# jiangzhengkai/mxdetection

Measured on AMD Instinct MI355X. Metric: images/sec (whole node) Faster R-CNN R50-FPN 3x800x1333, higher is better.
Workload: dtype bf16; 1 GPU; Faster R-CNN ResNet-50-FPN bf16 train step, batch 2/GPU, 3x800x1333 (padded 1344); global_batch=2, parallelism=dp1, frozen=stem+C2, frozen BN folded, optimizer=SGD momentum 0.9 wd 1e-4, launch=hipGraph replay, input=resident, wgrad_side_stream=True, rpn_branch_stream=True, grouped_wgrad=True, filter_prefetch_hints=True, params_trainable=41538304

## Files before the change

mxdetection_amd/csrc/boxes.hip:

```cpp
#include "common.h"

namespace mxdet {

__global__ void box_iou_kernel(const float4* __restrict__ a, int64_t na, const float4* __restrict__ b,
                               int64_t nb, float* __restrict__ out) {
  int64_t idx = (int64_t)blockIdx.x * blockDim.x + threadIdx.x;
  if (idx >= na * nb) return;
  int64_t i = idx / nb, j = idx - i * nb;
  float4 p = a[i], q = b[j];
  out[idx] = mxdet_iou(p.x, p.y, p.z, p.w, q.x, q.y, q.z, q.w);
}

__global__ void anchors_kernel(const float* __restrict__ base, int A, int H, int W, int stride,
                               float4* __restrict__ out) {
  int64_t idx = (int64_t)blockIdx.x * blockDim.x + threadIdx.x;
  int64_t total = (int64_t)H * W * A;
  if (idx >= total) return;
  int a = (int)(idx % A);
  int64_t cell = idx / A;
  int x = (int)(cell % W), y = (int)(cell / W);
  float sx = (float)(x * stride), sy = (float)(y * stride);
  float4 o;
  o.x = base[a * 4 + 0] + sx;
  o.y = base[a * 4 + 1] + sy;
  o.z = base[a * 4 + 2] + sx;
  o.w = base[a * 4 + 3] + sy;
  out[idx] = o;
}

__global__ void fpn_level_kernel(const float* __restrict__ rois, int64_t R, int lvl_min, int lvl_max,
                                 int32_t* __restrict__ levels) {
  int64_t i = (int64_t)blockIdx.x * blockDim.x + threadIdx.x;
  if (i >= R) return;
  const float* r = rois + i * 5;
  int k = mxdet_fpn_level(r[1], r[2], r[3], r[4]);
  k = k < lvl_min ? lvl_min : (k > lvl_max ? lvl_max : k);
  levels[i] = k;
}

__global__ void __launch_bounds__(64)
nms_mask_kernel(const float4* __restrict__ boxes, const int32_t* __restrict__ counts, int n_max,
                int nwords_max, float thresh, unsigned long long* __restrict__ mask) {
  const int col_blk = blockIdx.x, row_blk = blockIdx.y, b = blockIdx.z;
  if (col_blk < row_blk) return;
  int n = counts[b];
  n = n > n_max ? n_max : n;
  if (row_blk * 64 >= n || col_blk * 64 >= n) return;
  __shared__ float4 cb[64];
  const int t = threadIdx.x;
  const float4* bx = boxes + (int64_t)b * n_max;
  int cj = col_blk * 64 + t;
  if (cj < n) cb[t] = bx[cj];
  __syncthreads();
  int i = row_blk * 64 + t;
  if (i >= n) return;
  float4 r = bx[i];
  int ncol = n - col_blk * 64;
  ncol = ncol > 64 ? 64 : ncol;
  unsigned long long bits = 0;
  for (int j = 0; j < ncol; ++j) {
    int c = col_blk * 64 + j;
    float4 q = cb[j];
    float v = mxdet_iou(r.x, r.y, r.z, r.w, q.x, q.y, q.z, q.w);
    if (c > i && v > thresh) bits |= (1ull << j);
  }
  mask[((int64_t)b * n_max + i) * nwords_max + col_blk] = bits;
}

__device__ __forceinline__ unsigned long long readlane64(unsigned long long v, int lane) {
  unsigned lo = (unsigned)v, hi = (unsigned)(v >> 32);
  lo = (unsigned)__builtin_amdgcn_readlane((int)lo, lane);
  hi = (unsigned)__builtin_amdgcn_readlane((int)hi, lane);
  return ((unsigned long long)hi << 32) | lo;
}

__global__ void __launch_bounds__(64)
nms_scan_kernel(const unsigned long long* __restrict__ mask, const int32_t* __restrict__ counts,
                const uint8_t* __restrict__ invalid, int n_max, int nwords_max, int max_keep,
                int32_t* __restrict__ keep_idx, int32_t* __restrict__ num_keep) {
  __shared__ unsigned long long rem[64];
  const int b = blockIdx.x, lane = threadIdx.x;
  int n = counts[b];
  n = n > n_max ? n_max : n;
  n = __builtin_amdgcn_readfirstlane(n);
  const int nw = (n + 63) >> 6;
  const unsigned long long* m = mask + (int64_t)b * n_max * nwords_max;
  for (int w = 0; w < nw; ++w) {
    int idx = w * 64 + lane;
    bool bad = (idx >= n) || (invalid != nullptr && invalid[(int64_t)b * n_max + idx] != 0);
    unsigned long long bm = __ballot(bad);
    if (lane == 0) rem[w] = bm;
  }
  __syncthreads();
  unsigned long long mykeep = 0;
  unsigned long long diag_next = (nw > 0 && lane < n) ? m[(int64_t)lane * nwords_max] : 0ull;
  for (int w = 0; w < nw; ++w) {
    const unsigned long long diag = diag_next;
    if (w + 1 < nw) {
      int row = (w + 1) * 64 + lane;
      diag_next = (row < n) ? m[(int64_t)row * nwords_max + (w + 1)] : 0ull;
    }
    __syncthreads();
    unsigned long long cur = rem[w];
    cur = readlane64(cur, 0);
    unsigned long long keepbits = 0;
    for (int bb = 0; bb < 64; ++bb) {
      unsigned long long d = readlane64(diag, bb);
      if (!((cur >> bb) & 1ull)) {
        keepbits |= (1ull << bb);
        cur |= d;
      }
    }
    if (lane == w) mykeep = keepbits;
    if ((keepbits >> lane) & 1ull) {
      const unsigned long long* row = m + (int64_t)(w * 64 + lane) * nwords_max;
      for (int j = w + 1; j < nw; ++j) {
        unsigned long long v = row[j];
        if (v) atomicOr(&rem[j], v);
      }
    }
  }
  int cnt = __popcll(mykeep);
  int incl = cnt;
  for (int off = 1; off < 64; off <<= 1) {
    int v = __shfl_up(incl, off);
    if (lane >= off) incl += v;
  }
  int excl = incl - cnt;
  int total = __shfl(incl, 63);
  unsigned long long kb = mykeep;
  int pos = excl;
  while (kb) {
    int bb = __ffsll((long long)kb) - 1;
    kb &= kb - 1;
    if (pos < max_keep) keep_idx[(int64_t)b * n_max + pos] = lane * 64 + bb;
    ++pos;
  }
  if (lane == 0) num_keep[b] = total < max_keep ? total : max_keep;
}

template <int NW>
__global__ void __launch_bounds__(64)
nms_scan_rows_kernel(const unsigned long long* __restrict__ mask, const int32_t* __restrict__ counts,
                     const uint8_t* __restrict__ invalid, int n_max, int nwords_max, int max_keep,
                     int32_t* __restrict__ keep_idx, int32_t* __restrict__ num_keep) {
  __shared__ unsigned long long rows[2][64][NW + 1];
  const int b = blockIdx.x, lane = threadIdx.x;
  int n = counts[b];
  n = n > n_max ? n_max : n;
  n = __builtin_amdgcn_readfirstlane(n);
  const int nw = (n + 63) >> 6;
  const unsigned long long* m = mask + (int64_t)b * n_max * NW;
  unsigned long long myrem = 0ull;
  for (int w = 0; w < nw; ++w) {
    int idx = w * 64 + lane;
    bool bad = (idx >= n) || (invalid != nullptr && invalid[(int64_t)b * n_max + idx] != 0);
    unsigned long long bm = __ballot(bad);
    if (lane == w) myrem = bm;
  }
  unsigned long long nxt[NW];
  auto load_row = [&](unsigned long long (&r)[NW], int w) {
    const unsigned long long* bp = m + (int64_t)(w * 64) * NW + lane;
#pragma unroll
    for (int k = 0; k < NW; ++k) r[k] = bp[k * 64];
  };
  auto stage = [&](const unsigned long long (&r)[NW], int buf, int w) {
    unsigned long long* dst = &rows[buf][lane >> 5][lane & 31];
#pragma unroll
    for (int k = 0; k < NW; ++k) dst[k * 2 * (NW + 1)] = r[k];
  };
  load_row(nxt, 0);
  stage(nxt, 0, 0);
  __syncthreads();
  const int myword = lane < NW ? lane : 0;
  unsigned long long mykeep = 0;
  int buf = 0;
  for (int w = 0; w < nw; ++w) {
#ifndef NMS_ABL_NOLOAD
    if (w + 1 < nw) load_row(nxt, w + 1);
#endif
    const unsigned long long diag = rows[buf][lane][w];
    unsigned long long c = readlane64(myrem, w);
#ifndef NMS_ABL_NOCHAIN
#pragma unroll
    for (int bb = 0; bb < 64; ++bb) {
      unsigned long long d = readlane64(diag, bb);
      c |= ((c >> bb) & 1ull) ? 0ull : d;
    }
#else
    c |= readlane64(diag, 0);
#endif
    const unsigned long long keepbits = ~c;
    if (lane == w) mykeep = keepbits;
    const unsigned klo = __builtin_amdgcn_readfirstlane((unsigned)keepbits);
    const unsigned khi = __builtin_amdgcn_readfirstlane((unsigned)(keepbits >> 32));
    unsigned long long acc = 0ull;
#ifndef NMS_ABL_NOOR
#pragma unroll
#else
    if (klo == 0x12345u)
#endif
    for (int ch = 0; ch < 8; ++ch) {
      const unsigned bits = ((ch < 4 ? klo : khi) >> (8 * (ch & 3))) & 0xffu;
      if (bits == 0u) continue;
      unsigned long long v[8];
#pragma unroll
      for (int t = 0; t < 8; ++t) v[t] = rows[buf][8 * ch + t][myword];
#pragma unroll
      for (int t = 0; t < 8; ++t) acc |= ((bits >> t) & 1u) ? v[t] : 0ull;
    }
    if (lane > w && lane < nw) myrem |= acc;
    if (w + 1 < nw) stage(nxt, buf ^ 1, w + 1);
    __syncthreads();
    buf ^= 1;
  }
  int cnt = __popcll(mykeep);
  int incl = cnt;
  for (int off = 1; off < 64; off <<= 1) {
    int v = __shfl_up(incl, off);
    if (lane >= off) incl += v;
  }
  int excl = incl - cnt;
  int total = __shfl(incl, 63);
  unsigned long long kb = mykeep;
  int pos = excl;
  while (kb) {
    int bb = __ffsll((long long)kb) - 1;
    kb &= kb - 1;
    if (pos < max_keep) keep_idx[(int64_t)b * n_max + pos] = lane * 64 + bb;
    ++pos;
  }
  if (lane == 0) num_keep[b] = total < max_keep ? total : max_keep;
}

}

using namespace mxdet;

extern "C" int mxdet_box_iou(const float* boxes_a, int64_t na, const float* boxes_b, int64_t nb,
                             float* out, mxdet_stream_t stream) {
  clear_error();
  MXDET_REQUIRE(na >= 0 && nb >= 0, MXDET_ESHAPE, "box_iou: negative size");
  if (na == 0 || nb == 0) return MXDET_OK;
  MXDET_REQUIRE(boxes_a && boxes_b && out, MXDET_EINVAL, "box_iou: null pointer");
  int64_t total = na * nb;
  hipLaunchKernelGGL(box_iou_kernel, dim3((unsigned)ceil_div<int64_t>(total, 256)), dim3(256), 0,
                     as_stream(stream), (const float4*)boxes_a, na, (const float4*)boxes_b, nb, out);
  return check_launch("box_iou");
}

extern "C" int mxdet_generate_anchors(const float* base_anchors, int32_t A, int32_t H, int32_t W,
                                      int32_t stride, float* out, mxdet_stream_t stream) {
  clear_error();
  MXDET_REQUIRE(A > 0 && H >= 0 && W >= 0 && stride > 0, MXDET_ESHAPE, "generate_anchors: bad shape");
  int64_t total = (int64_t)H * W * A;
  if (total == 0) return MXDET_OK;
  MXDET_REQUIRE(base_anchors && out, MXDET_EINVAL, "generate_anchors: null pointer");
  hipLaunchKernelGGL(anchors_kernel, dim3((unsigned)ceil_div<int64_t>(total, 256)), dim3(256), 0,
                     as_stream(stream), base_anchors, A, H, W, stride, (float4*)out);
  return check_launch("generate_anchors");
}

extern "C" int mxdet_fpn_level_map(const float* rois, int64_t R, int32_t lvl_min, int32_t lvl_max,
                                   int32_t* levels, mxdet_stream_t stream) {
  clear_error();
  MXDET_REQUIRE(R >= 0 && lvl_min <= lvl_max, MXDET_ESHAPE, "fpn_level_map: bad arguments");
  if (R == 0) return MXDET_OK;
  MXDET_REQUIRE(rois && levels, MXDET_EINVAL, "fpn_level_map: null pointer");
  hipLaunchKernelGGL(fpn_level_kernel, dim3((unsigned)ceil_div<int64_t>(R, 256)), dim3(256), 0,
                     as_stream(stream), rois, R, lvl_min, lvl_max, levels);
  return check_launch("fpn_level_map");
}

extern "C" size_t mxdet_nms_batched_workspace_bytes(int32_t B, int32_t n_max) {
  if (B <= 0 || n_max <= 0) return 0;
  size_t nwords = (size_t)(n_max + 63) / 64;
  if (nwords <= 32) nwords = 32;
  return ((size_t)B * n_max + 64) * nwords * sizeof(unsigned long long);
}

extern "C" int mxdet_nms_batched(const float* boxes, const int32_t* counts, const uint8_t* invalid,
                                 int32_t B, int32_t n_max, float thresh, int32_t max_keep,
                                 int32_t* keep_idx, int32_t* num_keep, void* workspace,
                                 size_t workspace_bytes, mxdet_stream_t stream) {
  clear_error();
  MXDET_REQUIRE(B >= 0 && n_max >= 0, MXDET_ESHAPE, "nms_batched: negative size");
  if (B == 0) return MXDET_OK;
  MXDET_REQUIRE(n_max <= 4096, MXDET_ESHAPE, "nms_batched: n_max %d > 4096 unsupported", n_max);
  MXDET_REQUIRE(counts && num_keep, MXDET_EINVAL, "nms_batched: null pointer");
  if (n_max == 0) {
    hipError_t e = zero_async(num_keep, sizeof(int32_t) * B, as_stream(stream));
    MXDET_REQUIRE(e == hipSuccess, MXDET_EHIP, "nms_batched: memset failed");
    return MXDET_OK;
  }
  MXDET_REQUIRE(boxes && keep_idx, MXDET_EINVAL, "nms_batched: null pointer");
  size_t need = mxdet_nms_batched_workspace_bytes(B, n_max);
  MXDET_REQUIRE(workspace && workspace_bytes >= need, MXDET_EWORKSPACE,
                "nms_batched: workspace %zu < %zu", workspace_bytes, need);
  int nwords = (n_max + 63) / 64;
  const int pitch = nwords <= 32 ? 32 : nwords;
  hipLaunchKernelGGL(nms_mask_kernel, dim3(nwords, nwords, B), dim3(64), 0, as_stream(stream),
                     (const float4*)boxes, counts, n_max, pitch, thresh,
                     (unsigned long long*)workspace);
  if (nwords <= 32)
    hipLaunchKernelGGL(nms_scan_rows_kernel<32>, dim3(B), dim3(64), 0, as_stream(stream),
                       (const unsigned long long*)workspace, counts, invalid, n_max, nwords,
                       max_keep < 0 ? 0 : max_keep, keep_idx, num_keep);
  else
    hipLaunchKernelGGL(nms_scan_kernel, dim3(B), dim3(64), 0, as_stream(stream),
                       (const unsigned long long*)workspace, counts, invalid, n_max, nwords,
                       max_keep < 0 ? 0 : max_keep, keep_idx, num_keep);
  return check_launch("nms_batched");
}
```

Baseline: 471.8 images/sec.

## Speed up batched NMS with division-free IoU filter and four-wave scan

The NMS mask kernel now precomputes box areas and classifies most pairs with a division-free comparison of intersection against threshold-scaled union, using slightly widened bounds. Only pairs too close to the threshold fall back to the exact IoU. The scan kernel grows from one wave to four: wave 0 resolves the diagonal word with a split 32-bit chain plus DPP reduction, and all four waves share row loading and the OR-accumulation through shared memory. This adds block-wide barriers per word and extra shared memory, in exchange for less per-pair arithmetic and more parallel bandwidth in a step that is a small part of the training iteration.

```diff
diff --git a/mxdetection_amd/csrc/boxes.hip b/mxdetection_amd/csrc/boxes.hip
--- a/mxdetection_amd/csrc/boxes.hip
+++ b/mxdetection_amd/csrc/boxes.hip
@@ -38,32 +38,73 @@
   levels[i] = k;
 }
 
+__device__ __forceinline__ float vmax(float a, float b) {
+  float r;
+  asm("v_max_f32 %0, %1, %2" : "=v"(r) : "v"(a), "v"(b));
+  return r;
+}
+__device__ __forceinline__ float vmin(float a, float b) {
+  float r;
+  asm("v_min_f32 %0, %1, %2" : "=v"(r) : "v"(a), "v"(b));
+  return r;
+}
+
+__device__ __forceinline__ float nms_fast_area(float4 p) {
+  const float w = p.z - p.x + 1.0f, h = p.w - p.y + 1.0f;
+  const float lim = 1073741824.0f;
+  const bool ok = w > 0.0f && h > 0.0f && fabsf(p.x) <= lim && fabsf(p.y) <= lim && fabsf(p.z) <= lim && fabsf(p.w) <= lim;
+  return ok ? w * h : __builtin_nanf("");
+}
+
 __global__ void __launch_bounds__(64)
 nms_mask_kernel(const float4* __restrict__ boxes, const int32_t* __restrict__ counts, int n_max,
-                int nwords_max, float thresh, unsigned long long* __restrict__ mask) {
+                int nwords_max, float thresh, float t_hi, float t_lo, unsigned long long* __restrict__ mask) {
   const int col_blk = blockIdx.x, row_blk = blockIdx.y, b = blockIdx.z;
   if (col_blk < row_blk) return;
   int n = counts[b];
   n = n > n_max ? n_max : n;
   if (row_blk * 64 >= n || col_blk * 64 >= n) return;
   __shared__ float4 cb[64];
+  __shared__ float ca[64];
   const int t = threadIdx.x;
   const float4* bx = boxes + (int64_t)b * n_max;
   int cj = col_blk * 64 + t;
-  if (cj < n) cb[t] = bx[cj];
+  const float4 cq = cj < n ? bx[cj] : make_float4(0.0f, 0.0f, 0.0f, 0.0f);
+  cb[t] = cq;
+  ca[t] = nms_fast_area(cq);
   __syncthreads();
   int i = row_blk * 64 + t;
   if (i >= n) return;
-  float4 r = bx[i];
+  const float4 r = bx[i];
+  const float ar = nms_fast_area(r);
   int ncol = n - col_blk * 64;
   ncol = ncol > 64 ? 64 : ncol;
-  unsigned long long bits = 0;
-  for (int j = 0; j < ncol; ++j) {
-    int c = col_blk * 64 + j;
-    float4 q = cb[j];
-    float v = mxdet_iou(r.x, r.y, r.z, r.w, q.x, q.y, q.z, q.w);
-    if (c > i && v > thresh) bits |= (1ull << j);
-  }
+  auto half = [&](int j0) -> unsigned {
+    unsigned set = 0u, open = 0u;
+#pragma unroll 8
+    for (int j = 0; j < 32; ++j) {
+      const float4 q = cb[j0 + j];
+      const float iw = fmaxf(vmin(r.z, q.z) - vmax(r.x, q.x) + 1.0f, 0.0f);
+      const float ih = fmaxf(vmin(r.w, q.w) - vmax(r.y, q.y) + 1.0f, 0.0f);
+      const float inter = iw * ih;
+      float ua = ar + ca[j0 + j];
+      ua = ua - inter;
+      const bool above = inter > t_hi * ua, below = inter < t_lo * ua;
+      set |= above ? (1u << j) : 0u;
+      open |= (above || below) ? 0u : (1u << j);
+    }
+    while (open) {
+      const int j = __ffs((int)open) - 1;
+      open &= open - 1u;
+      const float4 q = cb[j0 + j];
+      if (mxdet_iou(r.x, r.y, r.z, r.w, q.x, q.y, q.z, q.w) > thresh) set |= 1u << j;
+    }
+    return set;
+  };
+  const unsigned lo = half(0), hi = half(32);
+  unsigned long long bits = ((unsigned long long)hi << 32) | lo;
+  if (col_blk == row_blk) bits &= ~((2ull << t) - 1ull);
+  if (ncol < 64) bits &= (1ull << ncol) - 1ull;
   mask[((int64_t)b * n_max + i) * nwords_max + col_blk] = bits;
 }
 
@@ -139,81 +180,125 @@
   if (lane == 0) num_keep[b] = total < max_keep ? total : max_keep;
 }
 
+__device__ __forceinline__ unsigned long long resolve_word(unsigned long long c, unsigned long long diag, int lane) {
+  const unsigned dlo = (unsigned)diag, dhi = (unsigned)(diag >> 32);
+  unsigned clo = (unsigned)c, chi = (unsigned)(c >> 32);
+#ifndef NMS_ABL_NOCHAIN
+#pragma unroll
+  for (int bb = 0; bb < 32; ++bb) {
+    const unsigned d = (unsigned)__builtin_amdgcn_readlane((int)dlo, bb);
+    clo |= ((clo >> bb) & 1u) ? 0u : d;
+  }
+  int v = (int)((lane < 32 && !((clo >> lane) & 1u)) ? dhi : 0u);
+  v |= __builtin_amdgcn_update_dpp(0, v, 0x128, 0xf, 0xf, false);
+  v |= __builtin_amdgcn_update_dpp(0, v, 0x124, 0xf, 0xf, false);
+  v |= __builtin_amdgcn_update_dpp(0, v, 0x122, 0xf, 0xf, false);
+  v |= __builtin_amdgcn_update_dpp(0, v, 0x121, 0xf, 0xf, false);
+  chi |= (unsigned)__builtin_amdgcn_readlane(v, 0) | (unsigned)__builtin_amdgcn_readlane(v, 16);
+#pragma unroll
+  for (int bb = 0; bb < 32; ++bb) {
+    const unsigned d = (unsigned)__builtin_amdgcn_readlane((int)dhi, 32 + bb);
+    chi |= ((chi >> bb) & 1u) ? 0u : d;
+  }
+#else
+  clo |= (unsigned)__builtin_amdgcn_readlane((int)dlo, 0);
+  chi |= (unsigned)__builtin_amdgcn_readlane((int)dhi, 0);
+#endif
+  return ((unsigned long long)chi << 32) | clo;
+}
+
 template <int NW>
-__global__ void __launch_bounds__(64)
+__global__ void __launch_bounds__(256)
 nms_scan_rows_kernel(const unsigned long long* __restrict__ mask, const int32_t* __restrict__ counts,
                      const uint8_t* __restrict__ invalid, int n_max, int nwords_max, int max_keep,
                      int32_t* __restrict__ keep_idx, int32_t* __restrict__ num_keep) {
+  static_assert(NW % 4 == 0 && 256 % NW == 0 && NW <= 64, "four waves share the 64 x NW words of a run evenly");
   __shared__ unsigned long long rows[2][64][NW + 1];
-  const int b = blockIdx.x, lane = threadIdx.x;
+  __shared__ unsigned long long part[3][64];
+  __shared__ unsigned long long kept_word;
+  __shared__ unsigned long long removed0[NW];
+  const int b = blockIdx.x, tid = threadIdx.x, lane = tid & 63;
+  const int wave = __builtin_amdgcn_readfirstlane(tid >> 6);
   int n = counts[b];
   n = n > n_max ? n_max : n;
   n = __builtin_amdgcn_readfirstlane(n);
   const int nw = (n + 63) >> 6;
   const unsigned long long* m = mask + (int64_t)b * n_max * NW;
-  unsigned long long myrem = 0ull;
-  for (int w = 0; w < nw; ++w) {
-    int idx = w * 64 + lane;
-    bool bad = (idx >= n) || (invalid != nullptr && invalid[(int64_t)b * n_max + idx] != 0);
-    unsigned long long bm = __ballot(bad);
-    if (lane == w) myrem = bm;
-  }
-  unsigned long long nxt[NW];
-  auto load_row = [&](unsigned long long (&r)[NW], int w) {
-    const unsigned long long* bp = m + (int64_t)(w * 64) * NW + lane;
-#pragma unroll
-    for (int k = 0; k < NW; ++k) r[k] = bp[k * 64];
+  constexpr int NQ = NW / 4;
+  unsigned long long nxt[NQ];
+  auto load_row = [&](unsigned long long (&r)[NQ], int w) {
+    const unsigned long long* bp = m + (int64_t)(w * 64) * NW + tid;
+#pragma unroll
+    for (int k = 0; k < NQ; ++k) r[k] = bp[k * 256];
   };
-  auto stage = [&](const unsigned long long (&r)[NW], int buf, int w) {
-    unsigned long long* dst = &rows[buf][lane >> 5][lane & 31];
-#pragma unroll
-    for (int k = 0; k < NW; ++k) dst[k * 2 * (NW + 1)] = r[k];
+  auto stage = [&](const unsigned long long (&r)[NQ], int buf) {
+    unsigned long long* dst = &rows[buf][tid / NW][tid % NW];
+#pragma unroll
+    for (int k = 0; k < NQ; ++k) dst[k * (256 / NW) * (NW + 1)] = r[k];
   };
   load_row(nxt, 0);
-  stage(nxt, 0, 0);
+  uint8_t flag[NQ];
+#pragma unroll
+  for (int k = 0; k < NQ; ++k) flag[k] = 0;
+  if (invalid != nullptr) {
+    const uint8_t* inv = invalid + (int64_t)b * n_max;
+#pragma unroll
+    for (int k = 0; k < NQ; ++k) {
+      const int idx = (wave * NQ + k) * 64 + lane;
+      flag[k] = inv[idx < n ? idx : 0];
+    }
+  }
+#pragma unroll
+  for (int k = 0; k < NQ; ++k) {
+    const int idx = (wave * NQ + k) * 64 + lane;
+    const unsigned long long bm = __ballot(idx >= n || flag[k] != 0);
+    if (lane == 0) removed0[wave * NQ + k] = bm;
+  }
+  stage(nxt, 0);
   __syncthreads();
   const int myword = lane < NW ? lane : 0;
+  const unsigned long long myrem0 = removed0[myword];
+  unsigned long long myrem = lane < nw ? myrem0 : 0ull;
   unsigned long long mykeep = 0;
   int buf = 0;
   for (int w = 0; w < nw; ++w) {
 #ifndef NMS_ABL_NOLOAD
     if (w + 1 < nw) load_row(nxt, w + 1);
 #endif
-    const unsigned long long diag = rows[buf][lane][w];
-    unsigned long long c = readlane64(myrem, w);
-#ifndef NMS_ABL_NOCHAIN
-#pragma unroll
-    for (int bb = 0; bb < 64; ++bb) {
-      unsigned long long d = readlane64(diag, bb);
-      c |= ((c >> bb) & 1ull) ? 0ull : d;
-    }
-#else
-    c |= readlane64(diag, 0);
-#endif
-    const unsigned long long keepbits = ~c;
-    if (lane == w) mykeep = keepbits;
-    const unsigned klo = __builtin_amdgcn_readfirstlane((unsigned)keepbits);
-    const unsigned khi = __builtin_amdgcn_readfirstlane((unsigned)(keepbits >> 32));
+    if (wave == 0) {
+      const unsigned long long diag = rows[buf][lane][w];
+      const unsigned long long keepbits = ~resolve_word(readlane64(myrem, w), diag, lane);
+      if (lane == w) mykeep = keepbits;
+      if (lane == 0) kept_word = keepbits;
+    }
+    __syncthreads();
+    const unsigned long long kw = kept_word;
+    const unsigned k16 = __builtin_amdgcn_readfirstlane((unsigned)(kw >> (16 * wave)));
     unsigned long long acc = 0ull;
 #ifndef NMS_ABL_NOOR
 #pragma unroll
 #else
-    if (klo == 0x12345u)
+    if (k16 == 0x12345u)
 #endif
-    for (int ch = 0; ch < 8; ++ch) {
-      const unsigned bits = ((ch < 4 ? klo : khi) >> (8 * (ch & 3))) & 0xffu;
+    for (int ch = 0; ch < 2; ++ch) {
+      const unsigned bits = (k16 >> (8 * ch)) & 0xffu;
       if (bits == 0u) continue;
       unsigned long long v[8];
 #pragma unroll
-      for (int t = 0; t < 8; ++t) v[t] = rows[buf][8 * ch + t][myword];
+      for (int t = 0; t < 8; ++t) v[t] = rows[buf][16 * wave + 8 * ch + t][myword];
 #pragma unroll
       for (int t = 0; t < 8; ++t) acc |= ((bits >> t) & 1u) ? v[t] : 0ull;
     }
-    if (lane > w && lane < nw) myrem |= acc;
-    if (w + 1 < nw) stage(nxt, buf ^ 1, w + 1);
+    if (wave != 0) part[wave - 1][lane] = acc;
+    if (w + 1 < nw) stage(nxt, buf ^ 1);
     __syncthreads();
+    if (wave == 0) {
+      acc |= part[0][lane] | part[1][lane] | part[2][lane];
+      if (lane > w && lane < nw) myrem |= acc;
+    }
     buf ^= 1;
   }
+  if (wave != 0) return;
   int cnt = __popcll(mykeep);
   int incl = cnt;
   for (int off = 1; off < 64; off <<= 1) {
@@ -299,11 +384,16 @@
                 "nms_batched: workspace %zu < %zu", workspace_bytes, need);
   int nwords = (n_max + 63) / 64;
   const int pitch = nwords <= 32 ? 32 : nwords;
+  float t_hi = INFINITY, t_lo = -INFINITY;
+  if (thresh == 0.0f || (fabsf(thresh) >= 0x1p-20f && fabsf(thresh) <= 0x1p20f)) {
+    t_hi = (float)((double)thresh * (1.0 + 0x1p-20));
+    t_lo = (float)((double)thresh * (1.0 - 0x1p-20));
+  }
   hipLaunchKernelGGL(nms_mask_kernel, dim3(nwords, nwords, B), dim3(64), 0, as_stream(stream),
-                     (const float4*)boxes, counts, n_max, pitch, thresh,
+                     (const float4*)boxes, counts, n_max, pitch, thresh, t_hi, t_lo,
                      (unsigned long long*)workspace);
   if (nwords <= 32)
-    hipLaunchKernelGGL(nms_scan_rows_kernel<32>, dim3(B), dim3(64), 0, as_stream(stream),
+    hipLaunchKernelGGL(nms_scan_rows_kernel<32>, dim3(B), dim3(256), 0, as_stream(stream),
                        (const unsigned long long*)workspace, counts, invalid, n_max, nwords,
                        max_keep < 0 ? 0 : max_keep, keep_idx, num_keep);
   else
```

Result: no change. 475.7 images/sec (median of 6 runs) (+0.8%).
